# Decade-qiu/Go2NetSpectra

Measured on AMD Instinct MI355X. Metric: Mpackets/s CMS update (device-resident, d=4 w=2^20) at 1/2/4/8 MI355X, higher is better.
Workload: dtype u32; 1 GPU; configs[1]: Count-Min d=4 w=2^20, 100M Zipf(1.1) 5-tuple headers in HBM per GPU, bit-exact counters; device_batch=100000000, key=5-tuple (37 B), parallelism=owner-key shards x1 (SrcIP slot; each GPU generates its shard of the stream), windows=steps use stream windows 0..619 (warmup first), none replayed

## Files before the change

go2netspectra_amd/csrc/gns_cm.hip:

```cpp
#include <algorithm>
#include <atomic>
#include <cstdlib>
#include <mutex>
#include <vector>

#include "gns_common.hpp"
#include "gns_ctl.cuh"
#include "gns_hh.hpp"
#include "gns_scan.cuh"
#include "gns_xcd.cuh"

namespace gns {

#ifndef GNS_TILE_BITS
#define GNS_TILE_BITS 12
#endif
#ifndef GNS_AP_THREADS
#define GNS_AP_THREADS 1024
#endif
#ifndef GNS_AP_ITEMS
#define GNS_AP_ITEMS 8
#endif
constexpr uint32_t kTileBitsMax = GNS_TILE_BITS;
constexpr uint32_t kTileMax = 1u << kTileBitsMax;
constexpr uint32_t kMaxTilesPerRow = 1024;
constexpr uint32_t kEntShift = 16;
constexpr uint32_t kSizeEsc = 0xFFFFu;
constexpr uint32_t kOvfFlag = 0x80000000u;
constexpr uint32_t kOvfCap = 1u << 20;
constexpr uint32_t kMaxBinsAll = 4096;
#ifndef GNS_EX_THREADS
#define GNS_EX_THREADS 256
#endif
constexpr int kExThreads = GNS_EX_THREADS;
constexpr size_t kExLdsSmall = 40 * 1024;
#ifndef GNS_CHUNK
#define GNS_CHUNK 16384
#endif
// ... 44 lines not shown
    const uint4 e = *reinterpret_cast<const uint4 *>(tabrow + hot_group(b) * 4);
    int h = -1;
    h = (e.w >> kHotBits) == b ? (int)(e.w & (kHot - 1u)) : h;
    h = (e.z >> kHotBits) == b ? (int)(e.z & (kHot - 1u)) : h;
    h = (e.y >> kHotBits) == b ? (int)(e.y & (kHot - 1u)) : h;
    h = (e.x >> kHotBits) == b ? (int)(e.x & (kHot - 1u)) : h;
    return h;
}

__device__ __forceinline__ uint32_t ceil_log2_dev(uint32_t x) { return x <= 1 ? 0u : 32u - __clz(x - 1u); }

__device__ __forceinline__ uint32_t row_index(const CmGeom &g, uint32_t h) {
    return g.pow2 ? (h & g.wmask) : (h % g.w);
}

struct HotSum {
    uint32_t n, nfc, nfs, smax;
    unsigned long long os, fs;
};

__host__ __device__ inline size_t extract_lds_bytes(uint32_t nbins_all, uint32_t d) {
    return (size_t)d * kHot * 16 + ((size_t)nbins_all + d * kHotTab) * 4 + (size_t)d * kHot * 20;
}

struct ExtractArgs {
    InputDesc in;
    uint64_t n;
    KeyPlanN kp;
    CmGeom g;
    DictDev D;
    uint32_t epoch;
    uint32_t *keyid;
    uint32_t *idx;
    uint64_t *pend;
    uint32_t *pend_cnt;
    uint32_t *pend_total;
    uint32_t *hist;
    uint32_t nblk;
    const uint32_t *hot_ids;
    const uint32_t *hot_tab;
    const uint32_t *Fc, *Fs;
    HotSum *hsum;
    unsigned long long *stats;
};

template <int KIND, int MODE>
__device__ __forceinline__ int packet_key(const InputDesc &in, uint32_t K, const uint8_t *s_src,
                                          uint64_t p, uint32_t (&kw)[GNS_KWMAX]) {
    if constexpr (KIND == IN_KEYS) {
        load_key_bytes<GNS_KWMAX>(in.keys + p * in.stride, K, (in.aligned & 1u) != 0, kw);
        return PARSE_OK;
    } else {
        uint32_t tw[10];
        const int st = load_tuple<KIND>(in, p, tw);
        if (st != PARSE_OK) return st;
        make_key_m<MODE, GNS_KWMAX>(K, s_src, tw, kw);
        return PARSE_OK;
    }
}

enum { CM_FOUND = 0, CM_PENDING = 1, CM_FULL = 2, CM_CLAIMED = 3 };

template <int N>
__device__ __forceinline__ int cm_find_or_claim(const DictDev &D, const uint32_t (&kw)[GNS_KWMAX], uint32_t K,
                                                uint32_t slot, uint32_t epoch, uint32_t *out,
                                                uint32_t (&r)[N]) {
// ... 92 lines not shown
            if (ok && (!cached || rr >= nc)) bk[rr] = row_index(a.g, mm3_chain<GNS_KWMAX>(mk, K, a.g.seeds[rr]));
        }
    }
    int hs[RMAX];
    bool anyhot = false;
#pragma unroll
    for (uint32_t rr = 0; rr < RMAX; rr++) {
        hs[rr] = -1;
        if (rr >= d) break;
        if (ok) hs[rr] = hot_lookup(s_tab + rr * kHotTab, bk[rr]);
        anyhot = anyhot || hs[rr] >= 0;
    }
    if (ok && first >= 2) {
        if (first == 2 || !anyhot) { res = CM_PENDING; out = first == 2 ? slot0 : ((slot0 + 1u) & a.D.mask); }
        else {
            res = cm_find_or_claim(a.D, kw, K, (slot0 + 1u) & a.D.mask, a.epoch, &out, rec);
            if (res == CM_CLAIMED) atomicAdd(S.s_claim, 1u);
        }
    }
    if (ok) {
        if (res == CM_FULL) {
            a.keyid[p] = GNS_ID_NONE;
            atomicAdd(&s_full, 1u);
            ok = false;
        } else if (res == CM_PENDING) {
            a.keyid[p] = GNS_ID_NONE;
            const uint32_t q = atomicAdd(&s_pend, 1u);
            a.pend[beg + q] = (uint64_t)(p - beg) << 32 | out;
        } else {
            a.keyid[p] = out;
            kid = out;
        }
    }

    if (bw && res == CM_CLAIMED) {
        uint32_t *tp = a.D.rec + (size_t)out * a.D.RW;
#pragma unroll
        for (uint32_t rr = 0; rr < RMAX; rr++)
            if (rr < d && rr < nc) tp[12 + rr] = bk[rr];
    }
    if (!ok) sz = 0;
    n_ok += (ok ? 1u : 0u) + (sz >= kSizeEsc ? 0x10000u : 0u);
#pragma unroll
    for (uint32_t rr = 0; rr < RMAX; rr++) {
        if (rr >= d) break;
        uint32_t binid = 0xFFFFFFFFu;
        int h = -1;
        if (ok) {
            const uint32_t b = bk[rr];
            h = hs[rr];
            a.idx[(uint64_t)rr * a.n + p] = h >= 0 ? (0x80000000u | (uint32_t)h) : b;
            binid = h >= 0 ? a.g.nbins + rr * kHot + (uint32_t)h : rr * a.g.ntiles + (b >> a.g.bin_bits);
        }
        const uint32_t b0 = __builtin_amdgcn_readfirstlane(binid);
        const uint64_t mm = __ballot(binid == b0 && b0 != 0xFFFFFFFFu);
        const uint32_t cnt = __popcll(mm);
        const bool agg = cnt >= 4;
        const bool inmaj = agg && binid == b0;
        const bool leader = inmaj && (uint32_t)__ffsll((long long)mm) - 1 == (threadIdx.x & 63u);
        if (leader) atomicAdd(&s_hist[b0], cnt);
        if (binid != 0xFFFFFFFFu && !inmaj) atomicAdd(&s_hist[binid], 1u);
        uint64_t ownv = 0;
        if (h >= 0) {
            const uint32_t slot = rr * kHot + (uint32_t)h;
            if (kid != s_hFc[slot]) atomicAdd(&s_nfc[slot], 1u);
            if (kid != s_hFs[slot]) {
                atomicAdd(&s_nfs[slot], 1u);
                atomicAdd(&s_fs[slot], (unsigned long long)sz);
                atomicMax(&s_smax[slot], sz);
            } else {
                ownv = sz;
            }
        }
        if (agg && b0 >= a.g.nbins && b0 != 0xFFFFFFFFu) {
            const uint64_t tot = wave_sum64(inmaj ? ownv : 0ull);
            if (leader && tot) atomicAdd(&s_os[b0 - a.g.nbins], (unsigned long long)tot);
            if (!inmaj && ownv) atomicAdd(&s_os[binid - a.g.nbins], (unsigned long long)ownv);
        } else if (ownv) {
            atomicAdd(&s_os[binid - a.g.nbins], (unsigned long long)ownv);
        }
    }
}

#ifndef GNS_EX_MINW
#define GNS_EX_MINW 4
#endif
#ifndef GNS_C5_THREADS
#define GNS_C5_THREADS 512
#endif
constexpr int kC5Threads = GNS_C5_THREADS;
#ifndef GNS_C5_PIPE
#define GNS_C5_PIPE 0
#endif
constexpr bool kC5Pipe = GNS_C5_PIPE != 0;
#ifndef GNS_C2_PIPE
#define GNS_C2_PIPE 1
#endif
constexpr bool kC2Pipe = GNS_C2_PIPE != 0;
template <int KIND, int MODE, int KB, int DD, int NT>
__global__ __launch_bounds__(NT, NT == 256 ? GNS_EX_MINW : (NT == 512 ? 2 : 1)) void k_extract(ExtractArgs a) {
    extern __shared__ __attribute__((aligned(16))) uint8_t xsm[];
    __shared__ uint32_t s_pend, s_drop, s_unsup, s_full, s_ok, s_claim;
    __shared__ uint8_t s_src[80];
    const uint32_t tid = threadIdx.x, blk = blockIdx.x;
    const uint32_t NS = a.g.d * kHot;
    unsigned long long *s_os = reinterpret_cast<unsigned long long *>(xsm);
    unsigned long long *s_fs = s_os + NS;
    uint32_t *s_tab = reinterpret_cast<uint32_t *>(s_fs + NS);
    uint32_t *s_hist = s_tab + a.g.d * kHotTab;
    uint32_t *s_hFc = s_hist + a.g.nbins_all;
    uint32_t *s_hFs = s_hFc + NS, *s_nfc = s_hFs + NS, *s_nfs = s_nfc + NS, *s_smax = s_nfs + NS;
    stage_plan<MODE>(a.kp, s_src);
    const uint32_t K = KB ? (uint32_t)KB : a.kp.K;
    const uint32_t d = DD ? (uint32_t)DD : a.g.d;
// ... 178 lines not shown
        if (r == CM_FOUND || r == CM_CLAIMED) {
            a.keyid[p] = out;
            if (r == CM_CLAIMED) atomicAdd(&s_claim, 1u);
            if (r == CM_CLAIMED && a.D.bw) {
                uint32_t mk[GNS_KWMAX];
                mm3_premix<GNS_KWMAX>(kw, a.kp.K, mk);
                uint32_t *tp = a.D.rec + (size_t)out * a.D.RW;
                const uint32_t nc = a.D.RW >= 32 ? 8u : 4u;
                for (uint32_t rr = 0; rr < nc && rr < a.g.d; rr++)
                    tp[12 + rr] = row_index(a.g, mm3_chain<GNS_KWMAX>(mk, a.kp.K, a.g.seeds[rr]));
            }
        } else if (r == CM_PENDING) {
            const uint32_t q = atomicAdd(&s_cnt, 1u);
            a.pend_out[beg + q] = (v & 0xFFFFFFFF00000000ull) | out;
        } else {
            atomicAdd(&s_full, 1u);
        }
    }
    __syncthreads();
    if (tid == 0) {
        a.cnt_out[blk] = s_cnt;
        if (s_cnt) atomicAdd(a.total_out, s_cnt);
        if (s_full) atomicAdd(&a.stats[3], (unsigned long long)s_full);
        dict_flush_claims(a.D, s_claim, &a.stats[3]);
    }
}


struct ScatterArgs {
    uint64_t n;
    CmGeom g;
    const uint32_t *keyid;
    const uint32_t *idx;
    const uint32_t *sizes;
    const uint32_t *offsets;
    uint32_t nblk;
    uint64_t *entries;
    uint64_t *ovf;
    uint32_t *ovf_cnt;
    uint32_t ovf_cap;
    const uint32_t *hot_ids;
    unsigned long long *stats;
    uint32_t hot_mode;
    const uint32_t *hflag2;
    const uint32_t *hany;
};

__host__ __device__ inline size_t scatter_lds_bytes(uint32_t LB, uint32_t d) {
    return (size_t)(2 * kScWaves + d) * LB * 4 + kScThreads * 4;
}

#ifdef GNS_K3_PROF
#define K3_MARK(i) do { if (threadIdx.x == 0) { const uint64_t tn_ = __builtin_amdgcn_s_memtime(); k3t[i] += tn_ - k3prev; k3prev = tn_; } } while (0)
#else
#define K3_MARK(i) do { } while (0)
#endif
template <int RANK>
__global__ __launch_bounds__(kScThreads) __attribute__((amdgpu_waves_per_eu(4))) void k_scatter(ScatterArgs a) {
#ifdef GNS_K3_PROF
    uint64_t k3t[5] = {0, 0, 0, 0, 0}, k3prev = __builtin_amdgcn_s_memtime();
#endif
    extern __shared__ __attribute__((aligned(16))) uint8_t smem[];
    const uint32_t LB = a.g.ntiles + kHot;
    const uint32_t d = a.g.d;
    uint32_t *s_cnt2 = reinterpret_cast<uint32_t *>(smem);
    uint32_t *s_goff = s_cnt2 + 2 * kScWaves * LB;
// ... 142 lines not shown
#pragma unroll
                    for (uint32_t w = 0; w < (uint32_t)kScWaves; w++) x[w] = s_cnt[w * LB + t];
                    uint32_t c = goff[t];
#pragma unroll
                    for (uint32_t w = 0; w < (uint32_t)kScWaves; w++) { s_cnt[w * LB + t] = c; c += x[w]; }
                    goff[t] = c;
                }
                for (uint32_t t = tid; t < kScWaves * LB; t += kScThreads) s_cnto[t] = 0;
            }
            __syncthreads();
            K3_MARK(2);
#pragma unroll
            for (int i = 0; i < kScItems; i++) asm volatile("" ::"v"(bsn[i]));
#pragma unroll
            for (int i = 0; i < kScItems; i++) {
                if ((br[i] >> 16) != 0xFFFFu) {
                    const uint32_t t = br[i] >> 16;
                    a.entries[s_cnt[wave * LB + t] + (br[i] & 0xFFFFu)] = ent[i];
                }
            }
            K3_MARK(4);
        }
    }
#ifdef GNS_K3_PROF
    if (threadIdx.x == 0 && !a.hot_mode) for (int i = 0; i < 5; i++) atomicAdd(&a.stats[kStatsProf + i], (unsigned long long)k3t[i]);
#endif
}

#ifndef GNS_ST_SUB
#define GNS_ST_SUB 8192
#endif
constexpr uint32_t kStSub = GNS_ST_SUB;
static_assert(kChunk % kStSub == 0, "whole sub-passes per K1 block");

constexpr int kStThreads = 1024;
template <int BINS, bool PK>
struct StLds {
    static constexpr int kWaves = kStThreads / 64;
    static constexpr int kCw = PK ? BINS / 2 : BINS;
    uint64_t stage[kStSub];
    uint16_t sbin[kStSub];
    uint32_t cnt[2][kWaves][kCw];
    uint32_t lstart[BINS], gpos[BINS];
    uint32_t goff[8][BINS];
    uint32_t wsum[BINS / 64];
    uint32_t dummy[kStThreads];
};

template <int BINS, bool PK>
__global__ __launch_bounds__(kStThreads) void k_scatter_st(ScatterArgs a) {
    static_assert(!PK || (kStSub / (kStThreads / 64) < 65536 && BINS % 128 == 0), "16-bit counter halves");
    constexpr uint32_t kCw = StLds<BINS, PK>::kCw;
    constexpr int kStWaves = kStThreads / 64;
    constexpr int kStItems = kStSub / kStThreads;
    constexpr uint32_t kStBins = BINS;
    static_assert(kStSub / kStWaves == kStItems * 64, "a wave owns kStItems x 64 consecutive packets of a sub-pass");
    static_assert(BINS <= kStThreads && BINS % 64 == 0, "one thread per bin in the bin scan");
    __shared__ StLds<BINS, PK> L;
#ifdef GNS_K3_PROF
    uint64_t k3t[5] = {0, 0, 0, 0, 0}, k3prev = __builtin_amdgcn_s_memtime();
#endif
    const uint32_t tid = threadIdx.x, lane = tid & 63u, wave = tid >> 6;
    const uint32_t d = a.g.d, nt = a.g.ntiles;
    const uint32_t blk = xcd_block(blockIdx.x, gridDim.x);
    const uint32_t tmask = (1u << a.g.bin_bits) - 1u;
    const uint64_t beg = (uint64_t)blk * kChunk;
    const uint64_t end = min(a.n, beg + kChunk);
    for (uint32_t i = tid; i < d * kStBins; i += kStThreads) {
        const uint32_t r = i / kStBins, t = i % kStBins;
        L.goff[r][t] = t < nt ? a.offsets[(uint64_t)blk * a.g.nbins_all + r * nt + t] : 0u;
    }
    for (uint32_t i = tid; i < 2 * kStWaves * kCw; i += kStThreads) (&L.cnt[0][0][0])[i] = 0;
    auto pkt = [&](uint64_t sp, int j) { return sp + (uint64_t)wave * (kStSub / kStWaves) + (uint64_t)j * 64 + lane; };
    uint32_t ids[kStItems], szs[kStItems], cds[kStItems];
    uint32_t ncd[kStItems], nids[kStItems], nszs[kStItems];
    auto load_ids = [&](uint64_t sp, uint32_t (&di)[kStItems], uint32_t (&ds)[kStItems]) {
#pragma unroll
        for (int j = 0; j < kStItems; j++) {
            const uint64_t p = pkt(sp, j);
            const uint64_t pc = p < end ? p : end - 1;
            di[j] = p < end ? a.keyid[pc] : GNS_ID_NONE;
            ds[j] = a.sizes[pc];
        }
    };
    auto load_codes = [&](uint64_t sp, uint32_t r, uint32_t (&c)[kStItems]) {
#pragma unroll
        for (int j = 0; j < kStItems; j++) {
            const uint64_t p = pkt(sp, j);
            c[j] = a.idx[(uint64_t)r * a.n + (p < end ? p : end - 1)];
        }
    };
    load_ids(beg, ids, szs);
    load_codes(beg, 0, cds);
    uint32_t par = 0;
    __syncthreads();
    for (uint64_t sp = beg; sp < end; sp += kStSub) {
        for (uint32_t r = 0; r < d; r++) {
            uint32_t (&cnt)[kStWaves][kCw] = L.cnt[par];
            K3_MARK(4);
            uint64_t ent[kStItems];
            uint32_t tb[kStItems];
#pragma unroll
            for (int j = 0; j < kStItems; j++) {
                const uint32_t b = cds[j];
                const bool valid = ids[j] != GNS_ID_NONE && (b >> 31) == 0;
                uint32_t t = 0xFFFFu, rk = 0;
                uint64_t e = 0;
                if (valid) {
                    t = b >> a.g.bin_bits;
                    const uint32_t low = b & tmask, sz = szs[j];
                    uint32_t lo = ids[j], sf = sz;
                    if (sz >= kSizeEsc) {
                        const uint32_t q = atomicAdd(a.ovf_cnt, 1u);
                        if (q < a.ovf_cap) {
                            a.ovf[q] = (uint64_t)sz << 32 | ids[j];
                            lo = kOvfFlag | q;
                        } else {
                            atomicAdd(&a.stats[4], 1ull);
                            lo = kOvfFlag | (a.ovf_cap - 1);
                        }
                        sf = kSizeEsc;
                    }
                    e = (uint64_t)((sf << kEntShift) | low) << 32 | lo;
                }
                ent[j] = e;
                tb[j] = t << 16 | rk;
            }
            {
                uint32_t rks[kStItems];
#pragma unroll
                for (int j = 0; j < kStItems; j++) {
                    const uint32_t t = tb[j] >> 16;
                    const uint32_t sh = PK && t != 0xFFFFu && t >= kCw ? 16u : 0u;
                    uint32_t *ad = t != 0xFFFFu ? &cnt[wave][PK ? t % kCw : t] : &L.dummy[tid];
                    rks[j] = atomicAdd(ad, t != 0xFFFFu ? 1u << sh : 0u);
                    if constexpr (PK) rks[j] = (rks[j] >> sh) & 0xFFFFu;
                }
#pragma unroll
                for (int j = 0; j < kStItems; j++) tb[j] |= rks[j];
            }
            const uint32_t r1 = r + 1 < d ? r + 1 : 0u;
            const uint64_t sp1 = r + 1 < d ? sp : sp + kStSub;
            if (sp1 < end) {
                load_codes(sp1, r1, ncd);
                if (r1 == 0) load_ids(sp1, nids, nszs);
            }
            __syncthreads();
            K3_MARK(0);
            uint32_t total = 0, incl = 0;
            if constexpr (PK) {
                if (tid < kCw) {
                    uint32_t r0 = 0, r1 = 0;
#pragma unroll
                    for (int w = 0; w < kStWaves; w++) {
                        const uint32_t x = cnt[w][tid];
                        cnt[w][tid] = r0 | r1 << 16;
                        r0 += x & 0xFFFFu;
                        r1 += x >> 16;
                    }
                    L.lstart[tid] = r0;
                    L.lstart[tid + kCw] = r1;
                }
                __syncthreads();
                if (tid < kStBins) {
                    total = L.lstart[tid];
                    incl = wave_incl_scan(total);
                    if (lane == 63) L.wsum[wave] = incl;
                }
            } else if (tid < kStBins) {
                const uint32_t t = tid;
                uint32_t run = 0;
                if (t < nt) {
#pragma unroll
                    for (int w = 0; w < kStWaves; w++) {
                        const uint32_t x = cnt[w][t];
                        cnt[w][t] = run;
                        run += x;
                    }
                }
                total = run;
                incl = wave_incl_scan(total);
                if (lane == 63) L.wsum[wave] = incl;
            }
            __syncthreads();
            if (tid < kStBins) {
                uint32_t base = 0;
#pragma unroll
                for (uint32_t w = 0; w < kStBins / 64; w++) base += w < wave ? L.wsum[w] : 0u;
                const uint32_t t = tid;
                L.lstart[t] = base + incl - total;
                L.gpos[t] = L.goff[r][t];
                L.goff[r][t] += total;
            }
            __syncthreads();
            K3_MARK(1);
#pragma unroll
            for (int j = 0; j < kStItems; j++) {
                const uint32_t t = tb[j] >> 16;
                if (t != 0xFFFFu) {
                    const uint32_t c = PK ? (cnt[wave][t % kCw] >> (t >= kCw ? 16u : 0u)) & 0xFFFFu : cnt[wave][t];
                    const uint32_t pos = L.lstart[t] + c + (tb[j] & 0xFFFFu);
                    L.stage[pos] = ent[j];
                    L.sbin[pos] = (uint16_t)t;
                }
            }
            __syncthreads();
            K3_MARK(2);
            if (sp1 < end) {
#pragma unroll
                for (int j = 0; j < kStItems; j++) cds[j] = ncd[j];
                if (r1 == 0) {
#pragma unroll
                    for (int j = 0; j < kStItems; j++) { ids[j] = nids[j]; szs[j] = nszs[j]; }
                }
            }
            uint32_t ntot = 0;
#pragma unroll
            for (uint32_t w = 0; w < kStBins / 64; w++) ntot += L.wsum[w];
            for (uint32_t i = tid; i < ntot; i += kStThreads) {
                const uint32_t t = L.sbin[i];
                a.entries[L.gpos[t] + (i - L.lstart[t])] = L.stage[i];
            }
            for (uint32_t i = tid; i < kStWaves * kCw; i += kStThreads) (&cnt[0][0])[i] = 0;
            par ^= 1u;
            K3_MARK(3);
        }
    }
#ifdef GNS_K3_PROF
    if (threadIdx.x == 0) for (int i = 0; i < 5; i++) atomicAdd(&a.stats[kStatsProf + i], (unsigned long long)k3t[i]);
#endif
}

__global__ __launch_bounds__(256) void k_lds_order_probe(uint32_t *viol, int iters) {
    __shared__ uint32_t s[4][64], s_old[4][64], s_ad[4][64];
    const uint32_t lane = threadIdx.x & 63u, w = threadIdx.x >> 6;
    uint32_t x = (blockIdx.x * 256 + threadIdx.x) * 0x9E3779B1u + 12345u, v = 0;
    for (int it = 0; it < iters; it++) {
        s[w][lane] = 0;
        x = x * 1664525u + 1013904223u;
        const uint32_t ad = (x >> 16) % (1u + (uint32_t)it % 16u);
        const uint32_t old = atomicAdd(&s[w][ad], 1u);
        s_old[w][lane] = old;
        s_ad[w][lane] = ad;
        for (uint32_t j = 0; j < lane; j++) v += (s_ad[w][j] == ad && s_old[w][j] >= old) ? 1u : 0u;
    }
    if (v) atomicAdd(viol, v);
}

__global__ __launch_bounds__(1024) void k_order(const uint32_t *offsets, uint32_t nblk, uint32_t nbins,
                                                uint32_t nall, const uint32_t *total, uint32_t *order) {
    constexpr uint32_t NK = 33 * 8;
    __shared__ uint32_t s_cnt[NK];
    __shared__ uint16_t s_key[4096];
    for (uint32_t k = threadIdx.x; k < NK; k += 1024) s_cnt[k] = 0;
    __syncthreads();
    for (uint32_t b = threadIdx.x; b < nbins; b += 1024) {
        const uint32_t s0 = offsets[b];
        const uint32_t s1 = (b + 1 < nall) ? offsets[b + 1] : *total;
        const uint32_t sz = s1 - s0;
        const uint32_t lz = __clz(sz);
        const uint32_t key = sz == 0 ? 0u : (32u - lz) * 8u + ((sz << lz) >> 28 & 7u);
        s_key[b] = (uint16_t)key;
// ... 1359 lines not shown
}

using namespace gns;

struct CmRead {
    HhScratch hh;
    uint8_t *qkeys = nullptr;
    uint64_t qkeys_n = 0;
    uint64_t *qout = nullptr;
    uint64_t qout_n = 0;
    void free_all() {
        hh.free_all();
        dfree(qkeys); dfree(qout);
        qkeys = nullptr; qout = nullptr;
        qkeys_n = qout_n = 0;
    }
};

struct gns_cm : FlowDict {
    int device = 0;
    hipStream_t stream = nullptr;
    CmGeom g{};
    KeyPlanN kp{};
    uint32_t K = 0, st = 0, ct = 0;
    uint32_t *C = nullptr, *S = nullptr, *Fc = nullptr, *Fs = nullptr;
    CmRead rd;
    std::atomic<uint32_t> period{0};
    std::mutex views_mu;
    std::vector<gns_cm_view *> views;
    uint32_t epoch = 0;
    uint64_t bmax = 0;
    uint32_t nblk_max = 0;
    uint32_t *keyid = nullptr, *idx = nullptr;
    uint64_t *pend[2] = {nullptr, nullptr};
    uint32_t *pcnt[2] = {nullptr, nullptr};
    uint32_t *ptotal = nullptr;
    uint32_t *hist = nullptr, *part = nullptr, *total = nullptr, *order = nullptr;
    uint64_t *entries = nullptr;
    uint32_t *rec_sizes = nullptr;
    uint64_t *ovf = nullptr;
    uint32_t *ovf_cnt = nullptr;
    uint64_t ovf_cap = 0;
    unsigned long long *stats = nullptr;
    uint32_t *hot_ids = nullptr;
    uint32_t *hot_tab = nullptr;
    long long *segtot = nullptr;
    uint32_t *hflag = nullptr, *hhist = nullptr, *hthr = nullptr, *hcnt = nullptr;
    uint32_t *hcand = nullptr, *hcn = nullptr;
    HotSum *hsum = nullptr;
    uint32_t *hflag2 = nullptr;
    uint32_t *work = nullptr;
    uint32_t ncu = 256;
    uint32_t *hres = nullptr;
    uint4 *chk = nullptr;
    bool warm = false;
    bool lds_ordered = false;
    uint32_t *h_pin = nullptr;
    HostStage stage[2];
    uint32_t *side_dev = nullptr;
    uint64_t side_n = 0;
    hipStream_t cstream = nullptr;
    hipEvent_t ev_copied[2] = {nullptr, nullptr}, ev_used[2] = {nullptr, nullptr};
    StageTimer timer;
};

struct gns_cm_view {
    gns_cm *cm = nullptr;
    hipStream_t stream = nullptr;
    hipEvent_t ready = nullptr;
    uint32_t *C = nullptr, *S = nullptr, *Fc = nullptr, *Fs = nullptr;
    CmRead rd;
    std::mutex mu;
    uint32_t period = ~0u;
};

struct ViewsQuiesced {
    std::unique_lock<std::mutex> reg;
    std::vector<std::unique_lock<std::mutex>> locks;
    explicit ViewsQuiesced(gns_cm *cm) : reg(cm->views_mu) {
        locks.reserve(cm->views.size());
        for (gns_cm_view *v : cm->views) locks.emplace_back(v->mu);
    }
};

namespace {

int cm_free_all(gns_cm *cm) {
    dfree(cm->C); dfree(cm->S); dfree(cm->Fc); dfree(cm->Fs); cm->rd.free_all();
    dfree(cm->keyid); dfree(cm->idx);
    dfree(cm->pend[0]); dfree(cm->pend[1]); dfree(cm->pcnt[0]); dfree(cm->pcnt[1]);
    dfree(cm->ptotal); dfree(cm->hist); dfree(cm->part); dfree(cm->total); dfree(cm->order);
    dfree(cm->entries); dfree(cm->rec_sizes); dfree(cm->ovf); dfree(cm->ovf_cnt); dfree(cm->stats);
    cm->stage[0].free_all(); cm->stage[1].free_all(); dfree(cm->side_dev);
    for (int i = 0; i < 2; i++) {
        if (cm->ev_copied[i]) (void)hipEventDestroy(cm->ev_copied[i]);
        if (cm->ev_used[i]) (void)hipEventDestroy(cm->ev_used[i]);
    }
    if (cm->cstream) (void)hipStreamDestroy(cm->cstream);
    dfree(cm->work);
    dfree(cm->hot_ids); dfree(cm->segtot); dfree(cm->hflag); dfree(cm->hhist); dfree(cm->hthr); dfree(cm->hcnt);
    dfree(cm->hcand); dfree(cm->hcn);
    dfree(cm->hsum); dfree(cm->hflag2); dfree(cm->hres); dfree(cm->chk); dfree(cm->hot_tab);
    cm->FlowDict::free_all();
    if (cm->h_pin) (void)hipHostFree(cm->h_pin);
    cm->timer.destroy();
    if (cm->stream) (void)hipStreamDestroy(cm->stream);
    return GNS_OK;
}

int cm_reset_state(gns_cm *cm) {
    const uint64_t cells = (uint64_t)cm->g.d * cm->g.w;
    GNS_HIP(hipMemsetAsync(cm->C, 0, cells * 4, cm->stream));
    GNS_HIP(hipMemsetAsync(cm->S, 0, cells * 4, cm->stream));
    GNS_HIP(hipMemsetAsync(cm->Fc, 0xFF, cells * 4, cm->stream));
    GNS_HIP(hipMemsetAsync(cm->Fs, 0xFF, cells * 4, cm->stream));
    GNS_HIP(hipMemsetAsync(cm->D.rec, 0, cm->dict_slots * cm->D.RW * 4, cm->stream));
    GNS_HIP(hipMemsetAsync(cm->hot_ids, 0xFF, (size_t)cm->g.d * kHot * 4, cm->stream));
    GNS_HIP(hipMemsetAsync(cm->hot_tab, 0xFF, (size_t)cm->g.d * kHotTab * 4, cm->stream));
    GNS_HIP(hipMemsetAsync(cm->hhist, 0, (size_t)cm->g.d * kHotKeys * 4, cm->stream));
    GNS_HIP(hipMemsetAsync(cm->hthr, 0xFF, 8 * 4, cm->stream));
    GNS_HIP(hipMemsetAsync(cm->hcn, 0, 16 * 4, cm->stream));
    GNS_HIP(hipMemsetAsync(cm->stats + 3, 0, 2 * sizeof(unsigned long long), cm->stream));
// ... 6 lines not shown

int cm_reclaim(gns_cm *cm, uint64_t min_slots = 0) {
    ViewsQuiesced q(cm);
    const uint64_t cells = (uint64_t)cm->g.d * cm->g.w;
    std::vector<DictIds> ids{{cm->Fc, cells}, {cm->Fs, cells}};
    const uint32_t period = cm->period.load();
    for (gns_cm_view *v : cm->views)
        if (v->period == period) { ids.push_back({v->Fc, cells}); ids.push_back({v->Fs, cells}); }
    return cm->reclaim(ids.data(), (int)ids.size(), min_slots, cm->stream);
}

template <int KIND, int MODE>
int cm_run_batch(gns_cm *cm, const InputDesc &in, uint64_t n) {
    if (n == 0) return GNS_OK;
    hipStream_t s = cm->stream;
    const uint32_t nblk = (uint32_t)((n + kChunk - 1) / kChunk);
    const CmGeom &g = cm->g;
    ScopedStage total_stage(cm->timer, 5);
    {
        CtlZero z;
        z.add(cm->ptotal, 8);
        z.add(cm->dctl + 1, 4);
        z.add(cm->hflag2, ((size_t)g.d * kHot + 2) * 4);
        z.add(cm->stats + 8, 8);
        z.add(cm->ovf_cnt, 4);
        z.add(cm->work, 4);
        z.add(cm->hflag, (size_t)g.d * kHot * 4);
        GNS_HIP(ctl_zero(z, s));
    }
    if (++cm->epoch == 0) cm->epoch = 1;
    {
        ExtractArgs a{};
        a.in = in; a.n = n; a.kp = cm->kp; a.g = g; a.D = cm->D; a.epoch = cm->epoch;
        a.keyid = cm->keyid; a.idx = cm->idx; a.pend = cm->pend[0]; a.pend_cnt = cm->pcnt[0];
        a.pend_total = cm->ptotal; a.hist = cm->hist; a.nblk = nblk; a.hot_ids = cm->hot_ids;
        a.Fc = cm->Fc; a.Fs = cm->Fs; a.hsum = cm->hsum; a.hot_tab = cm->hot_tab;
        a.stats = cm->stats;
        ScopedStage st(cm->timer, 0);
        const size_t lds = extract_lds_bytes(g.nbins_all, g.d);
        if constexpr (KIND == IN_REC16) {
            if (lds > kExLdsSmall)
                hipLaunchKernelGGL((k_extract<KIND, MODE, 0, 0, 1024>), dim3(nblk), dim3(1024), lds, s, a);
            else
                hipLaunchKernelGGL((k_extract<KIND, MODE, 0, 0, 256>), dim3(nblk), dim3(kExThreads), lds, s, a);
        } else if (lds > kExLdsSmall) {
            if (cm->K == 37 && g.d == 8)
                hipLaunchKernelGGL((k_extract<KIND, MODE, 37, 8, kC5Threads>), dim3(nblk), dim3(kC5Threads), lds, s, a);
            else if (cm->K == 37)
                hipLaunchKernelGGL((k_extract<KIND, MODE, 37, 0, 1024>), dim3(nblk), dim3(1024), lds, s, a);
            else if (cm->K == 16)
                hipLaunchKernelGGL((k_extract<KIND, MODE, 16, 0, 1024>), dim3(nblk), dim3(1024), lds, s, a);
            else
                hipLaunchKernelGGL((k_extract<KIND, MODE, 0, 0, 1024>), dim3(nblk), dim3(1024), lds, s, a);
        } else if (cm->K == 37 && g.d == 4)
            hipLaunchKernelGGL((k_extract<KIND, MODE, 37, 4, 256>), dim3(nblk), dim3(kExThreads), lds, s, a);
        else if (cm->K == 37)
            hipLaunchKernelGGL((k_extract<KIND, MODE, 37, 0, 256>), dim3(nblk), dim3(kExThreads), lds, s, a);
        else if (cm->K == 16 && g.d == 4)
            hipLaunchKernelGGL((k_extract<KIND, MODE, 16, 4, 256>), dim3(nblk), dim3(kExThreads), lds, s, a);
        else if (cm->K == 16)
            hipLaunchKernelGGL((k_extract<KIND, MODE, 16, 0, 256>), dim3(nblk), dim3(kExThreads), lds, s, a);
        else
            hipLaunchKernelGGL((k_extract<KIND, MODE, 0, 0, 256>), dim3(nblk), dim3(kExThreads), lds, s, a);
        GNS_HIP(hipGetLastError());
    }
    int cur = 0;
    for (int round = 0;; round++) {
// ... 21 lines not shown
                set_error("flow dictionary full (%llu slots); raise max_flows",
                          (unsigned long long)cm->dict_slots);
                return GNS_E_FULL;
            }
            if (cm->h_pin[0] == 0) break;
        }
        if (round > 64) { set_error("dictionary resolve did not converge"); return GNS_E_FULL; }
        if (++cm->epoch == 0) cm->epoch = 1;
        ResolveArgs a{};
        a.in = in; a.n = n; a.kp = cm->kp; a.D = cm->D; a.epoch = cm->epoch; a.keyid = cm->keyid;
        a.pend_in = cm->pend[cur]; a.cnt_in = cm->pcnt[cur];
        a.pend_out = cm->pend[cur ^ 1]; a.cnt_out = cm->pcnt[cur ^ 1]; a.total_out = cm->ptotal + (cur ^ 1);
        a.total_in = cm->ptotal + cur;
        a.stats = cm->stats; a.g = g;
        ScopedStage st(cm->timer, 1);
        hipLaunchKernelGGL((k_resolve<KIND, MODE>), dim3(nblk), dim3(kExThreads), 0, s, a);
        GNS_HIP(hipGetLastError());
        cur ^= 1;
    }
    {
        ScopedStage st(cm->timer, 2);
        const uint32_t ngrp = (nblk + kTGrp - 1) / kTGrp;
        const dim3 g2((g.nbins_all + 255) / 256, ngrp);
        uint32_t *tot = cm->part + (size_t)ngrp * g.nbins_all;
        hipLaunchKernelGGL(k_tscan_part, g2, dim3(256), 0, s, cm->hist, nblk, g.nbins_all, cm->part);
        hipLaunchKernelGGL(k_tscan_mid, dim3((g.nbins_all + 255) / 256), dim3(256), 0, s, cm->part, ngrp, g.nbins_all, tot);
        hipLaunchKernelGGL(k_tscan_bins, dim3(1), dim3(1024), 0, s, tot, g.nbins_all, cm->total);
        hipLaunchKernelGGL(k_tscan_down, g2, dim3(256), 0, s, cm->hist, nblk, g.nbins_all, cm->part, tot);
        GNS_HIP(hipGetLastError());
    }
    {
        ScatterArgs a{};
        a.n = n; a.g = g; a.keyid = cm->keyid; a.idx = cm->idx; a.sizes = in.sizes;
        a.offsets = cm->hist; a.nblk = nblk; a.entries = cm->entries; a.ovf = cm->ovf;
        a.ovf_cnt = cm->ovf_cnt; a.ovf_cap = (uint32_t)cm->ovf_cap; a.hot_ids = cm->hot_ids; a.stats = cm->stats;
        a.hot_mode = 0; a.hflag2 = cm->hflag2; a.hany = cm->hflag2 + g.d * kHot;
        ScopedStage st(cm->timer, 3);
        if (cm->lds_ordered && g.ntiles <= 256)
            hipLaunchKernelGGL((k_scatter_st<256, false>), dim3(nblk), dim3(kStThreads), 0, s, a);
        else if (cm->lds_ordered && g.ntiles <= 512)
            hipLaunchKernelGGL((k_scatter_st<512, true>), dim3(nblk), dim3(kStThreads), 0, s, a);
        else if (cm->lds_ordered)
            hipLaunchKernelGGL(k_scatter<1>, dim3(nblk), dim3(kScThreads), scatter_lds_bytes(g.ntiles + kHot, g.d), s, a);
        else
            hipLaunchKernelGGL(k_scatter<0>, dim3(nblk), dim3(kScThreads), scatter_lds_bytes(g.ntiles + kHot, g.d), s, a);
        GNS_HIP(hipGetLastError());
    }
    {
        const bool ordered = g.nbins <= 4096;
        if (ordered)
            hipLaunchKernelGGL(k_order, dim3(1), dim3(1024), 0, s, cm->hist, nblk, g.nbins, g.nbins_all,
                               cm->total, cm->order);
        ApplyArgs a{};
        a.stats = cm->stats;
        a.entries = cm->entries; a.offsets = cm->hist; a.nblk = nblk; a.nbins = g.nbins;
        a.total = cm->total; a.order = ordered ? cm->order : nullptr; a.ovf = cm->ovf; a.g = g;
        a.C = cm->C; a.Fc = cm->Fc; a.S = cm->S; a.Fs = cm->Fs; a.work = cm->work;
        ScopedStage st(cm->timer, 4);
        if (g.sub_bits) {
            const dim3 apg(std::min(g.nbins, cm->ncu));
            hipLaunchKernelGGL(k_apply_sparse, apg, dim3(kApThreads), 0, s, a);
        } else {
            const dim3 apg(std::min(g.nbins, cm->ncu * (kApThreads <= 512 ? 2u : 1u)));
            hipLaunchKernelGGL(k_apply, apg, dim3(kApThreads), 0, s, a);
        }
        GNS_HIP(hipGetLastError());
    }
// ... 202 lines not shown
        cm->timer.stream = cm->stream;
        {
            int ncu = 0;
            if (hipDeviceGetAttribute(&ncu, hipDeviceAttributeMultiprocessorCount, cm->device) == hipSuccess && ncu > 0)
                cm->ncu = (uint32_t)ncu;
        }
        const uint64_t cells = (uint64_t)g.d * g.w;
        if ((rc = dalloc_t(&cm->C, cells)) || (rc = dalloc_t(&cm->S, cells)) ||
            (rc = dalloc_t(&cm->Fc, cells)) || (rc = dalloc_t(&cm->Fs, cells)))
            break;
        const uint64_t mf = p->max_flows ? p->max_flows : (4ull << 20);
        uint64_t slots = 1;
        while (slots < 2 * mf) slots <<= 1;
        if (slots > kDictMaxSlots) { set_error("max_flows too large"); rc = GNS_E_ARG; break; }
        cm->dict_slots = slots;
        cm->max_flows = mf;
        cm->D.mask = (uint32_t)(slots - 1);
        cm->D.K = cm->K;
        cm->D.RW = dict_record_words_cm(cm->K, g.d);
        cm->D.bw = cm->D.RW >= 16 && 1 + (cm->K + 3) / 4 <= 12 ? 1u : 0u;
        cm->D.seed = 0x2545F491u;
        if ((rc = dalloc_t(&cm->D.rec, slots * cm->D.RW)) != GNS_OK) break;
        if ((rc = dalloc_t(&cm->dctl, 4)) != GNS_OK || (rc = dalloc_t(&cm->stats_bak, 3)) != GNS_OK) break;
        cm->D.ctl = cm->dctl;
        cm->limits();
        cm->bmax = p->batch_packets ? p->batch_packets : (16ull << 20);
        cm->bmax = ((cm->bmax + kChunk - 1) / kChunk) * kChunk;
        if (cm->bmax > (1ull << 31)) { set_error("batch_packets too large"); rc = GNS_E_ARG; break; }
        const uint64_t bcap = (((1ull << 31) / g.d) / kChunk) * kChunk;
        if (cm->bmax > bcap) cm->bmax = bcap;
        cm->nblk_max = (uint32_t)(cm->bmax / kChunk);
        const uint64_t nscan = ((uint64_t)(cm->nblk_max + kTGrp - 1) / kTGrp + 2) * g.nbins_all;
        if ((rc = dalloc_t(&cm->keyid, cm->bmax)) || (rc = dalloc_t(&cm->idx, cm->bmax * g.d)) ||
            (rc = dalloc_t(&cm->pend[0], cm->bmax)) || (rc = dalloc_t(&cm->pend[1], cm->bmax)) ||
            (rc = dalloc_t(&cm->pcnt[0], cm->nblk_max)) || (rc = dalloc_t(&cm->pcnt[1], cm->nblk_max)) ||
            (rc = dalloc_t(&cm->ptotal, 2)) || (rc = dalloc_t(&cm->hist, (uint64_t)g.nbins_all * cm->nblk_max)) ||
            (rc = dalloc_t(&cm->part, nscan)) || (rc = dalloc_t(&cm->total, 1)) ||
            (rc = dalloc_t(&cm->order, g.nbins)) || (rc = dalloc_t(&cm->entries, cm->bmax * g.d)) ||
            (rc = dalloc_t(&cm->ovf, kOvfCap)) || (rc = dalloc_t(&cm->ovf_cnt, 1)) ||
            (rc = dalloc_t(&cm->stats, kStatsProf + 16)) || (rc = dalloc_t(&cm->work, 1)) || (rc = dalloc_t(&cm->hot_ids, g.d * kHot)) ||
            (rc = dalloc_t(&cm->segtot, (size_t)g.d * kHot * kHotSegs * 2)) || (rc = dalloc_t(&cm->hflag, g.d * kHot)) ||
            (rc = dalloc_t(&cm->hhist, g.d * kHotKeys)) || (rc = dalloc_t(&cm->hthr, 8)) || (rc = dalloc_t(&cm->hcnt, 8)) ||
            (rc = dalloc_t(&cm->hcand, (size_t)g.d * kHotCand)) || (rc = dalloc_t(&cm->hcn, 16)) ||
            (rc = dalloc_t(&cm->hsum, (uint64_t)g.d * kHot * cm->nblk_max)) ||
            (rc = dalloc_t(&cm->hflag2, g.d * kHot + 2)) || (rc = dalloc_t(&cm->hres, g.d * kHot * 2)) ||
            (rc = dalloc_t(&cm->chk, kChkCap)) || (rc = dalloc_t(&cm->hot_tab, (size_t)g.d * kHotTab)))
            break;
        cm->ovf_cap = kOvfCap;
        if (hipHostMalloc(reinterpret_cast<void **>(&cm->h_pin), 64, 0) != hipSuccess) {
            set_error("hipHostMalloc failed"); rc = GNS_E_OOM; break;
        }
        if (hipMemsetAsync(cm->stats, 0, (kStatsProf + 16) * 8, cm->stream) != hipSuccess) { rc = GNS_E_HIP; break; }
        if ((rc = cm_reset_state(cm)) != GNS_OK) break;
        {
            const char *env = getenv("GNS_K3_RANK");
            uint32_t *viol = nullptr;
            if ((rc = dalloc_t(&viol, 1)) != GNS_OK) break;
            hipError_t e = hipMemsetAsync(viol, 0, 4, cm->stream);
            if (e == hipSuccess) {
                hipLaunchKernelGGL(k_lds_order_probe, dim3(4 * cm->ncu), dim3(256), 0, cm->stream, viol, 64);
                e = hipGetLastError();
            }
            uint32_t hv = 1;
            if (e == hipSuccess) e = hipMemcpyAsync(&hv, viol, 4, hipMemcpyDeviceToHost, cm->stream);
            if (e == hipSuccess) e = hipStreamSynchronize(cm->stream);
            dfree(viol);
// ... 366 lines not shown
int gns_cm_stats(gns_cm *cm, uint64_t stats[4]) {
    if (!cm || !stats) return GNS_E_ARG;
    GNS_TRY(set_device(cm->device));
    GNS_HIP(hipStreamSynchronize(cm->stream));
    unsigned long long h[8];
    GNS_HIP(hipMemcpy(h, cm->stats, sizeof(h), hipMemcpyDeviceToHost));
    stats[0] = h[0]; stats[1] = h[1]; stats[2] = h[2];
    std::vector<uint32_t> tags;
    uint64_t occ = 0;
    const uint64_t chunk = 1 << 20;
    std::vector<uint32_t> buf;
    for (uint64_t s0 = 0; s0 < cm->dict_slots; s0 += chunk) {
        const uint64_t m = std::min(chunk, cm->dict_slots - s0);
        buf.resize(m * cm->D.RW);
        GNS_HIP(hipMemcpy(buf.data(), cm->D.rec + s0 * cm->D.RW, m * cm->D.RW * 4, hipMemcpyDeviceToHost));
        for (uint64_t i = 0; i < m; i++) occ += buf[i * cm->D.RW] != 0;
    }
    stats[3] = occ;
    return GNS_OK;
}

int gns_cm_counters(gns_cm *cm, uint64_t out[8]) {
    if (!cm || !out) return GNS_E_ARG;
    GNS_TRY(set_device(cm->device));
    GNS_HIP(hipStreamSynchronize(cm->stream));
    unsigned long long h[kStatsProf + 16];
    GNS_HIP(hipMemcpy(h, cm->stats, sizeof(h), hipMemcpyDeviceToHost));
#if defined(GNS_SP_PROF)
    for (int i = 0; i < 7; i++) out[i] = h[kStatsProf + i];
    out[7] = h[6];
    return GNS_OK;
#endif
#ifdef GNS_K3_PROF
    for (int i = 0; i < 5; i++) out[i] = h[kStatsProf + i];
    for (int i = 5; i < 8; i++) out[i] = h[i];
    return GNS_OK;
#endif
#ifdef GNS_K4_PROF
    for (int i = 0; i < 4; i++) out[i] = h[kStatsProf + i];
    out[4] = h[kStatsProf + 9];
    out[5] = h[kStatsProf + 5];
    out[6] = h[kStatsProf + 8];
    out[7] = h[kStatsProf + 6];
#else
    for (int i = 0; i < 8; i++) out[i] = h[i];
#endif
    return GNS_OK;
}

int gns_cm_reclaim(gns_cm *cm) {
    if (!cm) return GNS_E_ARG;
    GNS_TRY(set_device(cm->device));
    return cm_reclaim(cm);
}

int gns_cm_dict_stats(gns_cm *cm, uint64_t out[8]) {
    if (!cm || !out) return GNS_E_ARG;
    out[0] = cm->n_reclaim; out[1] = cm->n_dropped; out[2] = cm->last_live; out[3] = cm->claimed;
    out[4] = (uint64_t)(cm->reclaim_ms * 1000.0); out[5] = cm->n_retry;
    out[6] = cm->dict_slots; out[7] = cm->n_grow;
    return GNS_OK;
}

int gns_cm_set_timing(gns_cm *cm, int on) {
    if (!cm) return GNS_E_ARG;
    set_timing_arg(cm->timer, on);
    return GNS_OK;
}
// ... 19 lines not shown
```

Baseline: 21300 Mpackets/s.

## Compact cold packets with per-wave bitmask so scatter skips hot-only packets

```diff
diff --git a/go2netspectra_amd/csrc/gns_cm.hip b/go2netspectra_amd/csrc/gns_cm.hip
--- a/go2netspectra_amd/csrc/gns_cm.hip
+++ b/go2netspectra_amd/csrc/gns_cm.hip
@@ -4,6 +4,7 @@
 #include <mutex>
 #include <vector>
 
+#include "gns_coldmask.cuh"
 #include "gns_common.hpp"
 #include "gns_ctl.cuh"
 #include "gns_hh.hpp"
@@ -114,6 +115,7 @@
     uint32_t epoch;
     uint32_t *keyid;
     uint32_t *idx;
+    uint64_t *cold;
     uint64_t *pend;
     uint32_t *pend_cnt;
     uint32_t *pend_total;
@@ -272,6 +274,7 @@
             kid = out;
         }
     }
+    uint64_t cmask = 0;
 
     if (bw && res == CM_CLAIMED) {
         uint32_t *tp = a.D.rec + (size_t)out * a.D.RW;
@@ -292,6 +295,7 @@
             a.idx[(uint64_t)rr * a.n + p] = h >= 0 ? (0x80000000u | (uint32_t)h) : b;
             binid = h >= 0 ? a.g.nbins + rr * kHot + (uint32_t)h : rr * a.g.ntiles + (b >> a.g.bin_bits);
         }
+        cmask |= __ballot(ok && h < 0);
         const uint32_t b0 = __builtin_amdgcn_readfirstlane(binid);
         const uint64_t mm = __ballot(binid == b0 && b0 != 0xFFFFFFFFu);
         const uint32_t cnt = __popcll(mm);
@@ -320,6 +324,7 @@
             atomicAdd(&s_os[binid - a.g.nbins], (unsigned long long)ownv);
         }
     }
+    if ((threadIdx.x & 63u) == 0 && p < a.n) a.cold[p >> 6] = cmask;
 }
 
 #ifndef GNS_EX_MINW
@@ -564,6 +569,7 @@
     CmGeom g;
     const uint32_t *keyid;
     const uint32_t *idx;
+    const uint64_t *cold;
     const uint32_t *sizes;
     const uint32_t *offsets;
     uint32_t nblk;
@@ -772,6 +778,8 @@
 #endif
 constexpr uint32_t kStSub = GNS_ST_SUB;
 static_assert(kChunk % kStSub == 0, "whole sub-passes per K1 block");
+constexpr uint32_t kStMaskW = kChunk / 64;
+static_assert(kStSub <= kColdNone && kChunk <= kColdNone, "16-bit packet offsets, kColdNone = none");
 
 constexpr int kStThreads = 1024;
 template <int BINS, bool PK>
@@ -785,6 +793,10 @@
     uint32_t goff[8][BINS];
     uint32_t wsum[BINS / 64];
     uint32_t dummy[kStThreads];
+    uint64_t cmask[kStMaskW];
+    uint32_t cpre[kStMaskW];
+    uint32_t cws[kStMaskW / 64];
+    uint16_t clist[kStSub];
 };
 
 template <int BINS, bool PK>
@@ -800,41 +812,77 @@
 #ifdef GNS_K3_PROF
     uint64_t k3t[5] = {0, 0, 0, 0, 0}, k3prev = __builtin_amdgcn_s_memtime();
 #endif
-    const uint32_t tid = threadIdx.x, lane = tid & 63u, wave = tid >> 6;
+    const uint32_t tid = threadIdx.x, lane = tid & 63u;
+    const uint32_t wave = __builtin_amdgcn_readfirstlane(tid >> 6);
     const uint32_t d = a.g.d, nt = a.g.ntiles;
     const uint32_t blk = xcd_block(blockIdx.x, gridDim.x);
     const uint32_t tmask = (1u << a.g.bin_bits) - 1u;
     const uint64_t beg = (uint64_t)blk * kChunk;
     const uint64_t end = min(a.n, beg + kChunk);
+    static_assert(kStMaskW <= kStThreads && kStMaskW % 64 == 0, "whole waves scan the mask words");
+    {
+        uint32_t pc = 0, incl = 0;
+        if (tid < kStMaskW) {
+            const uint32_t nw = (uint32_t)((end - beg + 63) >> 6);
+            const uint64_t m = tid < nw ? a.cold[(beg >> 6) + tid] : 0ull;
+            L.cmask[tid] = m;
+            pc = (uint32_t)__popcll(m);
+            incl = wave_incl_scan(pc);
+            if (lane == 63) L.cws[wave] = incl;
+        }
+        __syncthreads();
+        if (tid < kStMaskW) {
+            uint32_t base = 0;
+#pragma unroll
+            for (uint32_t w = 0; w < kStMaskW / 64; w++) base += w < wave ? L.cws[w] : 0u;
+            L.cpre[tid] = base + incl - pc;
+        }
+    }
+    uint32_t ncold = 0;
+#pragma unroll
+    for (uint32_t w = 0; w < kStMaskW / 64; w++) ncold += L.cws[w];
+    const uint32_t nsub = (ncold + kStSub - 1) / kStSub;
+    auto expand = [&](uint32_t k) {
+        cold_expand_lane(L.cmask, L.cpre, wave * (kStMaskW / kStWaves), (wave + 1) * (kStMaskW / kStWaves), lane,
+                         k * kStSub, kStSub, L.clist);
+    };
+    static_assert(kStMaskW % kStWaves == 0, "whole mask words per wave");
+    uint32_t ids[kStItems], szs[kStItems], cds[kStItems];
+    uint32_t ncd[kStItems], nids[kStItems], nszs[kStItems];
+    const uint32_t *kbase = a.keyid + beg, *sbase = a.sizes + beg;
+    auto load_step = [&](uint32_t k, uint32_t r, uint32_t (&c)[kStItems], uint32_t (&di)[kStItems],
+                         uint32_t (&ds)[kStItems]) {
+        const uint32_t *cbase = a.idx + ((uint64_t)r * a.n + beg);
+#pragma unroll
+        for (int j = 0; j < kStItems; j++) {
+            const uint32_t rk = wave * (kStSub / kStWaves) + (uint32_t)j * 64u + lane;
+            const bool has = k * kStSub + rk < ncold;
+            const uint32_t o = has ? (uint32_t)L.clist[rk] : 0u;
+            c[j] = cbase[o];
+            if (r == 0) {
+                di[j] = has ? kbase[o] : GNS_ID_NONE;
+                ds[j] = sbase[o];
+            }
+        }
+    };
+    __syncthreads();
+    if (nsub) {
+        expand(0);
+        __syncthreads();
+        load_step(0, 0, cds, ids, szs);
+    }
     for (uint32_t i = tid; i < d * kStBins; i += kStThreads) {
         const uint32_t r = i / kStBins, t = i % kStBins;
         L.goff[r][t] = t < nt ? a.offsets[(uint64_t)blk * a.g.nbins_all + r * nt + t] : 0u;
     }
     for (uint32_t i = tid; i < 2 * kStWaves * kCw; i += kStThreads) (&L.cnt[0][0][0])[i] = 0;
-    auto pkt = [&](uint64_t sp, int j) { return sp + (uint64_t)wave * (kStSub / kStWaves) + (uint64_t)j * 64 + lane; };
-    uint32_t ids[kStItems], szs[kStItems], cds[kStItems];
-    uint32_t ncd[kStItems], nids[kStItems], nszs[kStItems];
-    auto load_ids = [&](uint64_t sp, uint32_t (&di)[kStItems], uint32_t (&ds)[kStItems]) {
-#pragma unroll
-        for (int j = 0; j < kStItems; j++) {
-            const uint64_t p = pkt(sp, j);
-            const uint64_t pc = p < end ? p : end - 1;
-            di[j] = p < end ? a.keyid[pc] : GNS_ID_NONE;
-            ds[j] = a.sizes[pc];
-        }
-    };
-    auto load_codes = [&](uint64_t sp, uint32_t r, uint32_t (&c)[kStItems]) {
-#pragma unroll
-        for (int j = 0; j < kStItems; j++) {
-            const uint64_t p = pkt(sp, j);
-            c[j] = a.idx[(uint64_t)r * a.n + (p < end ? p : end - 1)];
-        }
-    };
-    load_ids(beg, ids, szs);
-    load_codes(beg, 0, cds);
+    if (d == 1 && nsub > 1) {
+        __syncthreads();
+        expand(1);
+    }
     uint32_t par = 0;
     __syncthreads();
-    for (uint64_t sp = beg; sp < end; sp += kStSub) {
+    for (uint32_t k = 0; k < nsub; k++) {
         for (uint32_t r = 0; r < d; r++) {
             uint32_t (&cnt)[kStWaves][kCw] = L.cnt[par];
             K3_MARK(4);
@@ -880,11 +928,9 @@
                 for (int j = 0; j < kStItems; j++) tb[j] |= rks[j];
             }
             const uint32_t r1 = r + 1 < d ? r + 1 : 0u;
-            const uint64_t sp1 = r + 1 < d ? sp : sp + kStSub;
-            if (sp1 < end) {
-                load_codes(sp1, r1, ncd);
-                if (r1 == 0) load_ids(sp1, nids, nszs);
-            }
+            const uint32_t k1 = r1 ? k : k + 1;
+            const bool more = k1 < nsub;
+            if (more) load_step(k1, r1, ncd, nids, nszs);
             __syncthreads();
             K3_MARK(0);
             uint32_t total = 0, incl = 0;
@@ -934,6 +980,7 @@
             }
             __syncthreads();
             K3_MARK(1);
+            if (more && r1 + 1 == d && k1 + 1 < nsub) expand(k1 + 1);
 #pragma unroll
             for (int j = 0; j < kStItems; j++) {
                 const uint32_t t = tb[j] >> 16;
@@ -946,7 +993,7 @@
             }
             __syncthreads();
             K3_MARK(2);
-            if (sp1 < end) {
+            if (more) {
 #pragma unroll
                 for (int j = 0; j < kStItems; j++) cds[j] = ncd[j];
                 if (r1 == 0) {
@@ -967,7 +1014,12 @@
         }
     }
 #ifdef GNS_K3_PROF
-    if (threadIdx.x == 0) for (int i = 0; i < 5; i++) atomicAdd(&a.stats[kStatsProf + i], (unsigned long long)k3t[i]);
+    if (threadIdx.x == 0) {
+        for (int i = 0; i < 5; i++) atomicAdd(&a.stats[kStatsProf + i], (unsigned long long)k3t[i]);
+        atomicAdd(&a.stats[kStatsProf + 5], (unsigned long long)ncold);
+        atomicMax(&a.stats[kStatsProf + 6], (unsigned long long)ncold);
+        if (nsub > 1) atomicAdd(&a.stats[kStatsProf + 7], 1ull);
+    }
 #endif
 }
 
@@ -2393,6 +2445,7 @@
     uint64_t bmax = 0;
     uint32_t nblk_max = 0;
     uint32_t *keyid = nullptr, *idx = nullptr;
+    uint64_t *cold = nullptr;
     uint64_t *pend[2] = {nullptr, nullptr};
     uint32_t *pcnt[2] = {nullptr, nullptr};
     uint32_t *ptotal = nullptr;
@@ -2448,7 +2501,7 @@
 
 int cm_free_all(gns_cm *cm) {
     dfree(cm->C); dfree(cm->S); dfree(cm->Fc); dfree(cm->Fs); cm->rd.free_all();
-    dfree(cm->keyid); dfree(cm->idx);
+    dfree(cm->keyid); dfree(cm->idx); dfree(cm->cold);
     dfree(cm->pend[0]); dfree(cm->pend[1]); dfree(cm->pcnt[0]); dfree(cm->pcnt[1]);
     dfree(cm->ptotal); dfree(cm->hist); dfree(cm->part); dfree(cm->total); dfree(cm->order);
     dfree(cm->entries); dfree(cm->rec_sizes); dfree(cm->ovf); dfree(cm->ovf_cnt); dfree(cm->stats);
@@ -2521,7 +2574,7 @@
     {
         ExtractArgs a{};
         a.in = in; a.n = n; a.kp = cm->kp; a.g = g; a.D = cm->D; a.epoch = cm->epoch;
-        a.keyid = cm->keyid; a.idx = cm->idx; a.pend = cm->pend[0]; a.pend_cnt = cm->pcnt[0];
+        a.keyid = cm->keyid; a.idx = cm->idx; a.cold = cm->cold; a.pend = cm->pend[0]; a.pend_cnt = cm->pcnt[0];
         a.pend_total = cm->ptotal; a.hist = cm->hist; a.nblk = nblk; a.hot_ids = cm->hot_ids;
         a.Fc = cm->Fc; a.Fs = cm->Fs; a.hsum = cm->hsum; a.hot_tab = cm->hot_tab;
         a.stats = cm->stats;
@@ -2609,7 +2662,7 @@
     {
         ScatterArgs a{};
         a.n = n; a.g = g; a.keyid = cm->keyid; a.idx = cm->idx; a.sizes = in.sizes;
-        a.offsets = cm->hist; a.nblk = nblk; a.entries = cm->entries; a.ovf = cm->ovf;
+        a.offsets = cm->hist; a.nblk = nblk; a.entries = cm->entries; a.ovf = cm->ovf; a.cold = cm->cold;
         a.ovf_cnt = cm->ovf_cnt; a.ovf_cap = (uint32_t)cm->ovf_cap; a.hot_ids = cm->hot_ids; a.stats = cm->stats;
         a.hot_mode = 0; a.hflag2 = cm->hflag2; a.hany = cm->hflag2 + g.d * kHot;
         ScopedStage st(cm->timer, 3);
@@ -2878,6 +2931,7 @@
         cm->nblk_max = (uint32_t)(cm->bmax / kChunk);
         const uint64_t nscan = ((uint64_t)(cm->nblk_max + kTGrp - 1) / kTGrp + 2) * g.nbins_all;
         if ((rc = dalloc_t(&cm->keyid, cm->bmax)) || (rc = dalloc_t(&cm->idx, cm->bmax * g.d)) ||
+            (rc = dalloc_t(&cm->cold, cm->bmax / 64)) ||
             (rc = dalloc_t(&cm->pend[0], cm->bmax)) || (rc = dalloc_t(&cm->pend[1], cm->bmax)) ||
             (rc = dalloc_t(&cm->pcnt[0], cm->nblk_max)) || (rc = dalloc_t(&cm->pcnt[1], cm->nblk_max)) ||
             (rc = dalloc_t(&cm->ptotal, 2)) || (rc = dalloc_t(&cm->hist, (uint64_t)g.nbins_all * cm->nblk_max)) ||
@@ -3310,8 +3364,7 @@
     return GNS_OK;
 #endif
 #ifdef GNS_K3_PROF
-    for (int i = 0; i < 5; i++) out[i] = h[kStatsProf + i];
-    for (int i = 5; i < 8; i++) out[i] = h[i];
+    for (int i = 0; i < 8; i++) out[i] = h[kStatsProf + i];
     return GNS_OK;
 #endif
 #ifdef GNS_K4_PROF
diff --git a/go2netspectra_amd/csrc/gns_coldmask.cuh b/go2netspectra_amd/csrc/gns_coldmask.cuh
--- /dev/null
+++ b/go2netspectra_amd/csrc/gns_coldmask.cuh
@@ -0,0 +1,29 @@
+#pragma once
+#include <stdint.h>
+
+#if defined(__HIPCC__)
+#include <hip/hip_runtime.h>
+#define GNS_CM_HD __host__ __device__ inline
+#else
+#define GNS_CM_HD inline
+#endif
+
+namespace gns {
+
+constexpr uint32_t kColdNone = 0xFFFFu;
+
+GNS_CM_HD uint32_t cold_rank(uint64_t word, uint32_t prefix, uint32_t l) {
+    return prefix + (uint32_t)__builtin_popcountll(word & ((1ull << l) - 1ull));
+}
+
+GNS_CM_HD void cold_expand_lane(const uint64_t *words, const uint32_t *prefix, uint32_t i0, uint32_t i1, uint32_t l,
+                                uint32_t lo, uint32_t cap, uint16_t *list) {
+#pragma unroll 1
+    for (uint32_t i = i0; i < i1; i++) {
+        const uint64_t w = words[i];
+        const uint32_t rk = cold_rank(w, prefix[i], l) - lo;
+        if (((w >> l) & 1ull) && rk < cap) list[rk] = (uint16_t)(64u * i + l);
+    }
+}
+
+}
```

After: 22830 Mpackets/s, median of 6. +7.1%, better.
